# mit-han-lab/duo-attention

Hardware: NVIDIA H100
Metric: decode tok/s @512K ctx (+ prefill tok/s @128K in `prefill`), Llama-3-8B, DuoAttention 50% retrieval heads (higher is better)
Workload: dtype bf16

## Files before the change

duo_attention_b200/csrc/attn_tc.cu:

```cuda
#include <cstdlib>

#include "duo_common.cuh"

namespace duo {

constexpr int TC_THREADS = 384;
constexpr int TC_TILE = 128;
constexpr int TC_BOX_BYTES = TC_TILE * 128;
constexpr int TC_TILE_BYTES = 2 * TC_BOX_BYTES;
constexpr int TC_MAX_W = 2048;
constexpr int TC_SMEM_BYTES = 5 * TC_TILE_BYTES + TC_MAX_W + 1024;

struct TcParams {
  void* out;
  long long out_batch_stride;
  int q_len, n_q_heads, group, n_full, n_stream, batch;
  int sink, recent, W;
  long long full_len, total, lo;
  float scale_log2;
  int cache_scan;
  int n_tok_tiles;
};

__device__ __forceinline__ void wg_fence() { asm volatile("wgmma.fence.sync.aligned;" ::: "memory"); }
__device__ __forceinline__ void wg_commit() { asm volatile("wgmma.commit_group.sync.aligned;" ::: "memory"); }
template <int N>
__device__ __forceinline__ void wg_wait() {
  asm volatile("wgmma.wait_group.sync.aligned %0;" ::"n"(N) : "memory");
}
__device__ __forceinline__ void wg_fence_regs(float (&d)[64]) {
#pragma unroll
  for (int i = 0; i < 64; ++i) asm volatile("" : "+f"(d[i])::"memory");
}

__device__ __forceinline__ uint64_t make_smem_desc(uint32_t saddr, uint32_t lbo_bytes, uint32_t sbo_bytes) {
  uint64_t d = 0;
  d |= (uint64_t)((saddr >> 4) & 0x3FFF);
  d |= (uint64_t)((lbo_bytes >> 4) & 0x3FFF) << 16;
  d |= (uint64_t)((sbo_bytes >> 4) & 0x3FFF) << 32;
  d |= 1ull << 62;
  return d;
}

template <bool BF16>
__device__ __forceinline__ void wgmma_ss(float (&d)[64], uint64_t adesc, uint64_t bdesc, uint32_t accum) {
  if constexpr (BF16) {
    asm volatile(
        "{\n\t.reg .pred p;\n\tsetp.ne.b32 p, %66, 0;\n\t"
        "wgmma.mma_async.sync.aligned.m64n128k16.f32.bf16.bf16 {%0,%1,%2,%3,%4,%5,%6,%7,%8,%9,%10,%11,%12,%13,%14,%15,%16,%17,%18,%19,%20,%21,%22,%23,%24,%25,%26,%27,%28,%29,%30,%31,%32,%33,%34,%35,%36,%37,%38,%39,%40,%41,%42,%43,%44,%45,%46,%47,%48,%49,%50,%51,%52,%53,%54,%55,%56,%57,%58,%59,%60,%61,%62,%63}, %64, %65, p, 1, 1, 0, 0;\n\t}"
        : "+f"(d[0]), "+f"(d[1]), "+f"(d[2]), "+f"(d[3]), "+f"(d[4]), "+f"(d[5]), "+f"(d[6]), "+f"(d[7]), "+f"(d[8]), "+f"(d[9]), "+f"(d[10]), "+f"(d[11]), "+f"(d[12]), "+f"(d[13]), "+f"(d[14]), "+f"(d[15]), "+f"(d[16]), "+f"(d[17]), "+f"(d[18]), "+f"(d[19]), "+f"(d[20]), "+f"(d[21]), "+f"(d[22]), "+f"(d[23]), "+f"(d[24]), "+f"(d[25]), "+f"(d[26]), "+f"(d[27]), "+f"(d[28]), "+f"(d[29]), "+f"(d[30]), "+f"(d[31]), "+f"(d[32]), "+f"(d[33]), "+f"(d[34]), "+f"(d[35]), "+f"(d[36]), "+f"(d[37]), "+f"(d[38]), "+f"(d[39]), "+f"(d[40]), "+f"(d[41]), "+f"(d[42]), "+f"(d[43]), "+f"(d[44]), "+f"(d[45]), "+f"(d[46]), "+f"(d[47]), "+f"(d[48]), "+f"(d[49]), "+f"(d[50]), "+f"(d[51]), "+f"(d[52]), "+f"(d[53]), "+f"(d[54]), "+f"(d[55]), "+f"(d[56]), "+f"(d[57]), "+f"(d[58]), "+f"(d[59]), "+f"(d[60]), "+f"(d[61]), "+f"(d[62]), "+f"(d[63])
        : "l"(adesc), "l"(bdesc), "r"(accum));
  } else {
    asm volatile(
        "{\n\t.reg .pred p;\n\tsetp.ne.b32 p, %66, 0;\n\t"
        "wgmma.mma_async.sync.aligned.m64n128k16.f32.f16.f16 {%0,%1,%2,%3,%4,%5,%6,%7,%8,%9,%10,%11,%12,%13,%14,%15,%16,%17,%18,%19,%20,%21,%22,%23,%24,%25,%26,%27,%28,%29,%30,%31,%32,%33,%34,%35,%36,%37,%38,%39,%40,%41,%42,%43,%44,%45,%46,%47,%48,%49,%50,%51,%52,%53,%54,%55,%56,%57,%58,%59,%60,%61,%62,%63}, %64, %65, p, 1, 1, 0, 0;\n\t}"
        : "+f"(d[0]), "+f"(d[1]), "+f"(d[2]), "+f"(d[3]), "+f"(d[4]), "+f"(d[5]), "+f"(d[6]), "+f"(d[7]), "+f"(d[8]), "+f"(d[9]), "+f"(d[10]), "+f"(d[11]), "+f"(d[12]), "+f"(d[13]), "+f"(d[14]), "+f"(d[15]), "+f"(d[16]), "+f"(d[17]), "+f"(d[18]), "+f"(d[19]), "+f"(d[20]), "+f"(d[21]), "+f"(d[22]), "+f"(d[23]), "+f"(d[24]), "+f"(d[25]), "+f"(d[26]), "+f"(d[27]), "+f"(d[28]), "+f"(d[29]), "+f"(d[30]), "+f"(d[31]), "+f"(d[32]), "+f"(d[33]), "+f"(d[34]), "+f"(d[35]), "+f"(d[36]), "+f"(d[37]), "+f"(d[38]), "+f"(d[39]), "+f"(d[40]), "+f"(d[41]), "+f"(d[42]), "+f"(d[43]), "+f"(d[44]), "+f"(d[45]), "+f"(d[46]), "+f"(d[47]), "+f"(d[48]), "+f"(d[49]), "+f"(d[50]), "+f"(d[51]), "+f"(d[52]), "+f"(d[53]), "+f"(d[54]), "+f"(d[55]), "+f"(d[56]), "+f"(d[57]), "+f"(d[58]), "+f"(d[59]), "+f"(d[60]), "+f"(d[61]), "+f"(d[62]), "+f"(d[63])
        : "l"(adesc), "l"(bdesc), "r"(accum));
  }
}
template <bool BF16>
__device__ __forceinline__ void wgmma_rs(float (&d)[64], const uint32_t* a, uint64_t bdesc) {
  if constexpr (BF16) {
    asm volatile(
        "{\n\t.reg .pred p;\n\tsetp.ne.b32 p, %69, 0;\n\t"
        "wgmma.mma_async.sync.aligned.m64n128k16.f32.bf16.bf16 {%0,%1,%2,%3,%4,%5,%6,%7,%8,%9,%10,%11,%12,%13,%14,%15,%16,%17,%18,%19,%20,%21,%22,%23,%24,%25,%26,%27,%28,%29,%30,%31,%32,%33,%34,%35,%36,%37,%38,%39,%40,%41,%42,%43,%44,%45,%46,%47,%48,%49,%50,%51,%52,%53,%54,%55,%56,%57,%58,%59,%60,%61,%62,%63}, {%64, %65, %66, %67}, %68, p, 1, 1, 1;\n\t}"
        : "+f"(d[0]), "+f"(d[1]), "+f"(d[2]), "+f"(d[3]), "+f"(d[4]), "+f"(d[5]), "+f"(d[6]), "+f"(d[7]), "+f"(d[8]), "+f"(d[9]), "+f"(d[10]), "+f"(d[11]), "+f"(d[12]), "+f"(d[13]), "+f"(d[14]), "+f"(d[15]), "+f"(d[16]), "+f"(d[17]), "+f"(d[18]), "+f"(d[19]), "+f"(d[20]), "+f"(d[21]), "+f"(d[22]), "+f"(d[23]), "+f"(d[24]), "+f"(d[25]), "+f"(d[26]), "+f"(d[27]), "+f"(d[28]), "+f"(d[29]), "+f"(d[30]), "+f"(d[31]), "+f"(d[32]), "+f"(d[33]), "+f"(d[34]), "+f"(d[35]), "+f"(d[36]), "+f"(d[37]), "+f"(d[38]), "+f"(d[39]), "+f"(d[40]), "+f"(d[41]), "+f"(d[42]), "+f"(d[43]), "+f"(d[44]), "+f"(d[45]), "+f"(d[46]), "+f"(d[47]), "+f"(d[48]), "+f"(d[49]), "+f"(d[50]), "+f"(d[51]), "+f"(d[52]), "+f"(d[53]), "+f"(d[54]), "+f"(d[55]), "+f"(d[56]), "+f"(d[57]), "+f"(d[58]), "+f"(d[59]), "+f"(d[60]), "+f"(d[61]), "+f"(d[62]), "+f"(d[63])
        : "r"(a[0]), "r"(a[1]), "r"(a[2]), "r"(a[3]), "l"(bdesc), "r"(1));
  } else {
    asm volatile(
        "{\n\t.reg .pred p;\n\tsetp.ne.b32 p, %69, 0;\n\t"
        "wgmma.mma_async.sync.aligned.m64n128k16.f32.f16.f16 {%0,%1,%2,%3,%4,%5,%6,%7,%8,%9,%10,%11,%12,%13,%14,%15,%16,%17,%18,%19,%20,%21,%22,%23,%24,%25,%26,%27,%28,%29,%30,%31,%32,%33,%34,%35,%36,%37,%38,%39,%40,%41,%42,%43,%44,%45,%46,%47,%48,%49,%50,%51,%52,%53,%54,%55,%56,%57,%58,%59,%60,%61,%62,%63}, {%64, %65, %66, %67}, %68, p, 1, 1, 1;\n\t}"
        : "+f"(d[0]), "+f"(d[1]), "+f"(d[2]), "+f"(d[3]), "+f"(d[4]), "+f"(d[5]), "+f"(d[6]), "+f"(d[7]), "+f"(d[8]), "+f"(d[9]), "+f"(d[10]), "+f"(d[11]), "+f"(d[12]), "+f"(d[13]), "+f"(d[14]), "+f"(d[15]), "+f"(d[16]), "+f"(d[17]), "+f"(d[18]), "+f"(d[19]), "+f"(d[20]), "+f"(d[21]), "+f"(d[22]), "+f"(d[23]), "+f"(d[24]), "+f"(d[25]), "+f"(d[26]), "+f"(d[27]), "+f"(d[28]), "+f"(d[29]), "+f"(d[30]), "+f"(d[31]), "+f"(d[32]), "+f"(d[33]), "+f"(d[34]), "+f"(d[35]), "+f"(d[36]), "+f"(d[37]), "+f"(d[38]), "+f"(d[39]), "+f"(d[40]), "+f"(d[41]), "+f"(d[42]), "+f"(d[43]), "+f"(d[44]), "+f"(d[45]), "+f"(d[46]), "+f"(d[47]), "+f"(d[48]), "+f"(d[49]), "+f"(d[50]), "+f"(d[51]), "+f"(d[52]), "+f"(d[53]), "+f"(d[54]), "+f"(d[55]), "+f"(d[56]), "+f"(d[57]), "+f"(d[58]), "+f"(d[59]), "+f"(d[60]), "+f"(d[61]), "+f"(d[62]), "+f"(d[63])
        : "r"(a[0]), "r"(a[1]), "r"(a[2]), "r"(a[3]), "l"(bdesc), "r"(1));
  }
}

template <typename T>
struct TcType;
template <>
struct TcType<__nv_bfloat16> {
  static constexpr bool bf16 = true;
  __device__ static uint32_t pack(float a, float b) {
    __nv_bfloat162 v = __floats2bfloat162_rn(a, b);
    return *reinterpret_cast<uint32_t*>(&v);
  }
};
template <>
struct TcType<__half> {
  static constexpr bool bf16 = false;
  __device__ static uint32_t pack(float a, float b) {
    __half2 v = __floats2half2_rn(a, b);
    return *reinterpret_cast<uint32_t*>(&v);
  }
};

struct TcBarriers {
  uint64_t q_full;
  uint64_t k_full[2], k_empty[2], v_full[2], v_empty[2];
};

template <typename T>
__global__ void __launch_bounds__(TC_THREADS, 1)
duo_attn_tc_kernel(const __grid_constant__ CUtensorMap map_q, const __grid_constant__ CUtensorMap map_fk,
                   const __grid_constant__ CUtensorMap map_fv, const __grid_constant__ CUtensorMap map_rk,
                   const __grid_constant__ CUtensorMap map_rv, const TcParams p) {
  extern __shared__ __align__(1024) uint8_t smem_raw[];
  uint8_t* smem = reinterpret_cast<uint8_t*>((reinterpret_cast<uintptr_t>(smem_raw) + 1023) & ~uintptr_t(1023));
  __shared__ TcBarriers bars;

  uint8_t* sQ = smem;
  uint8_t* sK = smem + 1 * TC_TILE_BYTES;
  uint8_t* sV = smem + 3 * TC_TILE_BYTES;
  uint8_t* sValid = smem + 5 * TC_TILE_BYTES;

  const int tid = threadIdx.x;
  const int b = blockIdx.y;

  int x = blockIdx.x;
  const int per_kvh = p.group * p.n_tok_tiles;
  const int kvh = x / per_kvh;
  x -= kvh * per_kvh;
  const int qh = kvh * p.group + x / p.n_tok_tiles;
  const int tok0 = (p.n_tok_tiles - 1 - (x % p.n_tok_tiles)) * TC_TILE;
  const bool is_full = kvh < p.n_full;
  const int tok_hi = min(p.q_len, tok0 + TC_TILE);
  long long a0 = 0, a1, b0 = 0, b1 = 0, base;
  if (is_full) {
    base = p.full_len;
    a1 = p.full_len + tok_hi;
  } else {
    base = p.W;
    a1 = p.cache_scan;
    b0 = p.W;
    b1 = (long long)p.W + tok_hi;
  }
  const int nA = (int)((a1 - a0 + TC_TILE - 1) / TC_TILE);
  const int nB = (int)((b1 - b0 + TC_TILE - 1) / TC_TILE);
  const int n_tiles = nA + nB;
  const CUtensorMap* mk = is_full ? &map_fk : &map_rk;
  const CUtensorMap* mv = is_full ? &map_fv : &map_rv;
  const int head_coord = is_full ? (b * p.n_full + kvh) : (b * p.n_stream + (kvh - p.n_full));
  auto tile_start = [&](int i) -> long long {
    return i < nA ? a0 + (long long)i * TC_TILE : b0 + (long long)(i - nA) * TC_TILE;
  };

  if (tid == 0) {
    prefetch_tmap(&map_q);
    prefetch_tmap(mk);
    prefetch_tmap(mv);
    mbar_init(&bars.q_full, 1);
    for (int s = 0; s < 2; ++s) {
      mbar_init(&bars.k_full[s], 1);
      mbar_init(&bars.k_empty[s], 256);
      mbar_init(&bars.v_full[s], 1);
      mbar_init(&bars.v_empty[s], 256);
    }
    fence_barrier_init();
  }
  if (!is_full) {
    for (int j = tid; j < p.W; j += TC_THREADS) sValid[j] = stream_slot_valid(j, p.sink, p.recent, p.total, p.lo) ? 1 : 0;
  }
  __syncthreads();

  if (tid < 128) {
    asm volatile("setmaxnreg.dec.sync.aligned.u32 24;");
    if (tid == 0) {
      mbar_expect_tx(&bars.q_full, TC_TILE_BYTES);
      tma_load_3d(sQ, &map_q, &bars.q_full, qh * kHeadDim, tok0, b);
      tma_load_3d(sQ + TC_BOX_BYTES, &map_q, &bars.q_full, qh * kHeadDim + 64, tok0, b);
      for (int j = 0; j < n_tiles; ++j) {
        const int st = j & 1;
        const uint32_t ph = (j >> 1) & 1;
        const int j0 = (int)tile_start(j);
        mbar_wait(&bars.k_empty[st], ph ^ 1);
        mbar_expect_tx(&bars.k_full[st], TC_TILE_BYTES);
        tma_load_3d(sK + st * TC_TILE_BYTES, mk, &bars.k_full[st], 0, j0, head_coord);
        tma_load_3d(sK + st * TC_TILE_BYTES + TC_BOX_BYTES, mk, &bars.k_full[st], 64, j0, head_coord);
        mbar_wait(&bars.v_empty[st], ph ^ 1);
        mbar_expect_tx(&bars.v_full[st], TC_TILE_BYTES);
        tma_load_3d(sV + st * TC_TILE_BYTES, mv, &bars.v_full[st], 0, j0, head_coord);
        tma_load_3d(sV + st * TC_TILE_BYTES + TC_BOX_BYTES, mv, &bars.v_full[st], 64, j0, head_coord);
      }
    }
    return;
  }

  asm volatile("setmaxnreg.inc.sync.aligned.u32 240;");
  constexpr bool kBf16 = TcType<T>::bf16;
  const int wg = (tid >> 7) - 1;
  const int wt = tid & 127;
  const int quad = wt & 3;
  const int row0 = wg * 64 + (wt >> 5) * 16 + ((wt & 31) >> 2);
  const float c = p.scale_log2;
  const long long min_limit = base + tok0 + wg * 64;
  int tok[2];
  bool row_ok[2];
  long long limit[2];
#pragma unroll
  for (int i = 0; i < 2; ++i) {
    tok[i] = tok0 + row0 + 8 * i;
    row_ok[i] = tok[i] < p.q_len;
    limit[i] = base + tok[i];
  }

  const uint32_t q_addr = smem_u32(sQ) + wg * 64 * 128, k_addr = smem_u32(sK), v_addr = smem_u32(sV);
  auto issue_s = [&](float (&s)[64], int st) {
    const uint32_t ka = k_addr + st * TC_TILE_BYTES;
#pragma unroll
    for (int kk = 0; kk < 8; ++kk) {
      const uint32_t off = (kk >> 2) * TC_BOX_BYTES + (kk & 3) * 32;
      wgmma_ss<kBf16>(s, make_smem_desc(q_addr + off, 16, 1024), make_smem_desc(ka + off, 16, 1024), kk > 0);
    }
  };
  auto issue_pv = [&](float (&o)[64], const uint32_t (&pk)[32], int st) {
    const uint32_t va = v_addr + st * TC_TILE_BYTES;
#pragma unroll
    for (int kk = 0; kk < 8; ++kk) wgmma_rs<kBf16>(o, &pk[4 * kk], make_smem_desc(va + kk * 2048, TC_BOX_BYTES, 1024));
  };

  float s[64], o[64];
#pragma unroll
  for (int i = 0; i < 64; ++i) o[i] = 0.f;
  float m_run[2] = {-INFINITY, -INFINITY};
  float l_run[2] = {0.f, 0.f};

  mbar_wait(&bars.q_full, 0);
  mbar_wait(&bars.k_full[0], 0);
  wg_fence();
  issue_s(s, 0);
  wg_commit();
  wg_wait<0>();
  wg_fence_regs(s);
  mbar_arrive(&bars.k_empty[0]);

  for (int j = 0; j < n_tiles; ++j) {
    const int st = j & 1;
    const uint32_t ph = (j >> 1) & 1;
    const long long j0 = tile_start(j);
    const long long jend = (j < nA) ? a1 : b1;
    const bool cache_seg = (!is_full) && (j < nA);
    const bool need_mask = cache_seg || (j0 + TC_TILE > jend) || (j0 + TC_TILE - 1 > min_limit);
    if (need_mask) {
#pragma unroll
      for (int nb = 0; nb < 16; ++nb) {
#pragma unroll
        for (int e = 0; e < 2; ++e) {
          const long long jj = j0 + nb * 8 + quad * 2 + e;
          bool slot_ok = jj < jend;
          if (cache_seg) slot_ok = slot_ok && (jj < p.W) && (sValid[jj < p.W ? jj : 0] != 0);
#pragma unroll
          for (int i = 0; i < 2; ++i)
            if (!(slot_ok && row_ok[i] && jj <= limit[i])) s[nb * 4 + 2 * i + e] = -INFINITY;
        }
      }
    }
    uint32_t pk[32];
#pragma unroll
    for (int i = 0; i < 2; ++i) {
      float mx = -INFINITY;
#pragma unroll
      for (int nb = 0; nb < 16; ++nb) mx = fmaxf(mx, fmaxf(s[nb * 4 + 2 * i], s[nb * 4 + 2 * i + 1]));
      mx = fmaxf(mx, __shfl_xor_sync(0xffffffffu, mx, 1));
      mx = fmaxf(mx, __shfl_xor_sync(0xffffffffu, mx, 2));
      const float m_new = fmaxf(m_run[i], mx);
      const float alpha = (m_new == -INFINITY) ? 1.f : fast_exp2((m_run[i] - m_new) * c);
      const float mref_c = (m_new == -INFINITY) ? 0.f : m_new * c;
      m_run[i] = m_new;
      float rs = 0.f;
#pragma unroll
      for (int nb = 0; nb < 16; ++nb) {
        const float p0 = fast_exp2(__fmaf_rn(s[nb * 4 + 2 * i], c, -mref_c));
        const float p1 = fast_exp2(__fmaf_rn(s[nb * 4 + 2 * i + 1], c, -mref_c));
        rs += p0 + p1;
        pk[nb * 2 + i] = TcType<T>::pack(p0, p1);
        o[nb * 4 + 2 * i] *= alpha;
        o[nb * 4 + 2 * i + 1] *= alpha;
      }
      l_run[i] = l_run[i] * alpha + rs;
    }
    mbar_wait_spin(&bars.v_full[st], ph);
    wg_fence();
    issue_pv(o, pk, st);
    wg_commit();
    const bool more = j + 1 < n_tiles;
    if (more) {
      const int st1 = (j + 1) & 1;
      mbar_wait_spin(&bars.k_full[st1], ((j + 1) >> 1) & 1);
      wg_fence();
      issue_s(s, st1);
      wg_commit();
    }
    wg_wait<0>();
    wg_fence_regs(o);
    wg_fence_regs(s);
    mbar_arrive(&bars.v_empty[st]);
    if (more) mbar_arrive(&bars.k_empty[(j + 1) & 1]);
  }

  T* out_b = reinterpret_cast<T*>(p.out) + (long long)b * p.out_batch_stride;
#pragma unroll
  for (int i = 0; i < 2; ++i) {
    float l = l_run[i];
    l += __shfl_xor_sync(0xffffffffu, l, 1);
    l += __shfl_xor_sync(0xffffffffu, l, 2);
    const float inv = l > 0.f ? 1.f / l : 0.f;
    if (row_ok[i]) {
      T* dst = out_b + ((long long)tok[i] * p.n_q_heads + qh) * kHeadDim + quad * 2;
#pragma unroll
      for (int nb = 0; nb < 16; ++nb)
        *reinterpret_cast<uint32_t*>(dst + nb * 8) = TcType<T>::pack(o[nb * 4 + 2 * i] * inv, o[nb * 4 + 2 * i + 1] * inv);
    }
  }
}

typedef CUresult (*EncodeTiledFn)(CUtensorMap*, CUtensorMapDataType, cuuint32_t, void*, const cuuint64_t*,
                                  const cuuint64_t*, const cuuint32_t*, const cuuint32_t*, CUtensorMapInterleave,
                                  CUtensorMapSwizzle, CUtensorMapL2promotion, CUtensorMapFloatOOBfill);
EncodeTiledFn get_encode_fn();

bool tc_prefill_supported(const duo_layer* L, const duo_cache_state* st, int q_len) {
  (void)st;
  if (L->d.kv_format != DUO_KV_SAME) return false;
  if (q_len < TC_TILE) return false;
  if (L->d.sink + L->d.recent > TC_MAX_W) return false;
  return true;
}

int launch_attn_tc(const duo_layer* L, const duo_cache_state* st, const void* q, long long q_row_stride, void* out,
                   int q_len, float scale, cudaStream_t stream) {
  const duo_layer_desc& d = L->d;
  EncodeTiledFn fn = get_encode_fn();
  if (!fn) return DUO_ECUDA;
  CUtensorMap map_q;
  {
    cuuint64_t dims[3] = {(cuuint64_t)q_row_stride, (cuuint64_t)q_len, (cuuint64_t)d.batch};
    cuuint64_t strides[2] = {(cuuint64_t)q_row_stride * 2, (cuuint64_t)q_row_stride * 2 * (cuuint64_t)q_len};
    cuuint32_t box[3] = {64, TC_TILE, 1};
    cuuint32_t estr[3] = {1, 1, 1};
    CUresult r = fn(&map_q, d.dtype == DUO_DT_BF16 ? CU_TENSOR_MAP_DATA_TYPE_BFLOAT16 : CU_TENSOR_MAP_DATA_TYPE_FLOAT16, 3,
                    const_cast<void*>(q), dims, strides, box, estr, CU_TENSOR_MAP_INTERLEAVE_NONE,
                    CU_TENSOR_MAP_SWIZZLE_128B, CU_TENSOR_MAP_L2_PROMOTION_L2_256B, CU_TENSOR_MAP_FLOAT_OOB_FILL_NONE);
    if (r != CUDA_SUCCESS) {
      set_error("cuTensorMapEncodeTiled(q) failed with CUresult %d", (int)r);
      return DUO_ECUDA;
    }
  }
  TcParams p{};
  p.out = out;
  const int n_q = (d.n_full + d.n_stream) * d.group;
  p.out_batch_stride = (long long)q_len * n_q * kHeadDim;
  p.q_len = q_len;
  p.n_q_heads = n_q;
  p.group = d.group;
  p.n_full = d.n_full;
  p.n_stream = d.n_stream;
  p.batch = d.batch;
  p.sink = d.sink;
  p.recent = d.recent;
  p.W = d.sink + d.recent;
  p.full_len = st->full_len;
  p.total = st->total;
  p.lo = st->lo;
  p.scale_log2 = scale * 1.4426950408889634f;
  p.cache_scan = (int)std::min<long long>(p.W, st->total);
  p.n_tok_tiles = (q_len + TC_TILE - 1) / TC_TILE;
  const int grid_x = n_q * p.n_tok_tiles;
  const CUtensorMap& fk = L->has_full_maps ? L->maps.full_k128 : L->maps.ring_k128;
  const CUtensorMap& fv = L->has_full_maps ? L->maps.full_v128 : L->maps.ring_v128;
  const CUtensorMap& rk = L->has_ring_maps ? L->maps.ring_k128 : L->maps.full_k128;
  const CUtensorMap& rv = L->has_ring_maps ? L->maps.ring_v128 : L->maps.full_v128;
  if (d.dtype == DUO_DT_BF16) {
    auto kern = duo_attn_tc_kernel<__nv_bfloat16>;
    static unsigned long long attr_mask = 0;
    if (int rc = ensure_dyn_smem(kern, TC_SMEM_BYTES, &attr_mask)) return rc;
    kern<<<dim3(grid_x, d.batch), TC_THREADS, TC_SMEM_BYTES, stream>>>(map_q, fk, fv, rk, rv, p);
  } else {
    auto kern = duo_attn_tc_kernel<__half>;
    static unsigned long long attr_mask = 0;
    if (int rc = ensure_dyn_smem(kern, TC_SMEM_BYTES, &attr_mask)) return rc;
    kern<<<dim3(grid_x, d.batch), TC_THREADS, TC_SMEM_BYTES, stream>>>(map_q, fk, fv, rk, rv, p);
  }
  DUO_CUDA_TRY(cudaGetLastError());
  return DUO_OK;
}

}
```

Before: 56.49.

## Pingpong warpgroups with named barriers and overlap QK^T with PV in prefill kernel

Restructures the tensor-core prefill attention loop into a FlashAttention-3 style schedule. Each warpgroup now issues S=QK^T for tile j together with PV for tile j-1 and runs the softmax of tile j while the PV wgmma is still in flight. Named barriers alternate the two consumer warpgroups so one issues MMAs while the other does softmax. Block-to-head mapping is also changed so that consecutive blocks share the same token tile across query heads of a group, which may improve L2 reuse of K/V. The cost is more live registers (P held in s plus pk) and more complex barrier and phase bookkeeping. Decode throughput is mostly unaffected since this kernel serves prefill.

```diff
diff --git a/duo_attention_b200/csrc/attn_tc.cu b/duo_attention_b200/csrc/attn_tc.cu
--- a/duo_attention_b200/csrc/attn_tc.cu
+++ b/duo_attention_b200/csrc/attn_tc.cu
@@ -32,6 +32,8 @@
 #pragma unroll
   for (int i = 0; i < 64; ++i) asm volatile("" : "+f"(d[i])::"memory");
 }
+__device__ __forceinline__ void named_bar_sync(int id) { asm volatile("bar.sync %0, 256;" ::"r"(id) : "memory"); }
+__device__ __forceinline__ void named_bar_arrive(int id) { asm volatile("bar.arrive %0, 256;" ::"r"(id) : "memory"); }
 
 __device__ __forceinline__ uint64_t make_smem_desc(uint32_t saddr, uint32_t lbo_bytes, uint32_t sbo_bytes) {
   uint64_t d = 0;
@@ -120,8 +122,8 @@
   const int per_kvh = p.group * p.n_tok_tiles;
   const int kvh = x / per_kvh;
   x -= kvh * per_kvh;
-  const int qh = kvh * p.group + x / p.n_tok_tiles;
-  const int tok0 = (p.n_tok_tiles - 1 - (x % p.n_tok_tiles)) * TC_TILE;
+  const int qh = kvh * p.group + x % p.group;
+  const int tok0 = (p.n_tok_tiles - 1 - x / p.group) * TC_TILE;
   const bool is_full = kvh < p.n_full;
   const int tok_hi = min(p.q_len, tok0 + TC_TILE);
   long long a0 = 0, a1, b0 = 0, b1 = 0, base;
@@ -219,23 +221,14 @@
   };
 
   float s[64], o[64];
+  uint32_t pk[32];
 #pragma unroll
   for (int i = 0; i < 64; ++i) o[i] = 0.f;
   float m_run[2] = {-INFINITY, -INFINITY};
   float l_run[2] = {0.f, 0.f};
-
-  mbar_wait(&bars.q_full, 0);
-  mbar_wait(&bars.k_full[0], 0);
-  wg_fence();
-  issue_s(s, 0);
-  wg_commit();
-  wg_wait<0>();
-  wg_fence_regs(s);
-  mbar_arrive(&bars.k_empty[0]);
-
-  for (int j = 0; j < n_tiles; ++j) {
-    const int st = j & 1;
-    const uint32_t ph = (j >> 1) & 1;
+  float alpha[2];
+
+  auto softmax = [&](int j) {
     const long long j0 = tile_start(j);
     const long long jend = (j < nA) ? a1 : b1;
     const bool cache_seg = (!is_full) && (j < nA);
@@ -254,7 +247,6 @@
         }
       }
     }
-    uint32_t pk[32];
 #pragma unroll
     for (int i = 0; i < 2; ++i) {
       float mx = -INFINITY;
@@ -263,7 +255,7 @@
       mx = fmaxf(mx, __shfl_xor_sync(0xffffffffu, mx, 1));
       mx = fmaxf(mx, __shfl_xor_sync(0xffffffffu, mx, 2));
       const float m_new = fmaxf(m_run[i], mx);
-      const float alpha = (m_new == -INFINITY) ? 1.f : fast_exp2((m_run[i] - m_new) * c);
+      alpha[i] = (m_new == -INFINITY) ? 1.f : fast_exp2((m_run[i] - m_new) * c);
       const float mref_c = (m_new == -INFINITY) ? 0.f : m_new * c;
       m_run[i] = m_new;
       float rs = 0.f;
@@ -272,29 +264,74 @@
         const float p0 = fast_exp2(__fmaf_rn(s[nb * 4 + 2 * i], c, -mref_c));
         const float p1 = fast_exp2(__fmaf_rn(s[nb * 4 + 2 * i + 1], c, -mref_c));
         rs += p0 + p1;
-        pk[nb * 2 + i] = TcType<T>::pack(p0, p1);
-        o[nb * 4 + 2 * i] *= alpha;
-        o[nb * 4 + 2 * i + 1] *= alpha;
+        s[nb * 4 + 2 * i] = p0;
+        s[nb * 4 + 2 * i + 1] = p1;
       }
-      l_run[i] = l_run[i] * alpha + rs;
-    }
-    mbar_wait_spin(&bars.v_full[st], ph);
-    wg_fence();
-    issue_pv(o, pk, st);
-    wg_commit();
-    const bool more = j + 1 < n_tiles;
-    if (more) {
-      const int st1 = (j + 1) & 1;
-      mbar_wait_spin(&bars.k_full[st1], ((j + 1) >> 1) & 1);
-      wg_fence();
-      issue_s(s, st1);
-      wg_commit();
-    }
+      l_run[i] = l_run[i] * alpha[i] + rs;
+    }
+  };
+  auto rescale_pack = [&]() {
+#pragma unroll
+    for (int nb = 0; nb < 16; ++nb) {
+#pragma unroll
+      for (int i = 0; i < 2; ++i) {
+        pk[nb * 2 + i] = TcType<T>::pack(s[nb * 4 + 2 * i], s[nb * 4 + 2 * i + 1]);
+        o[nb * 4 + 2 * i] *= alpha[i];
+        o[nb * 4 + 2 * i + 1] *= alpha[i];
+      }
+    }
+  };
+  const int bar_mine = 1 + wg, bar_other = 2 - wg;
+
+  mbar_wait(&bars.q_full, 0);
+  mbar_wait(&bars.k_full[0], 0);
+  if (wg == 1) named_bar_sync(bar_mine);
+  wg_fence();
+  issue_s(s, 0);
+  wg_commit();
+  named_bar_arrive(bar_other);
+  wg_wait<0>();
+  wg_fence_regs(s);
+  mbar_arrive(&bars.k_empty[0]);
+  softmax(0);
+
+  auto retire_pv = [&](int j) {
     wg_wait<0>();
     wg_fence_regs(o);
+    if (j > 1) mbar_arrive(&bars.v_empty[j & 1]);
+    rescale_pack();
+  };
+
+  for (int j = 1; j < n_tiles; ++j) {
+    const int st = j & 1, pst = st ^ 1;
+    retire_pv(j);
+    mbar_wait_spin(&bars.k_full[st], (j >> 1) & 1);
+    mbar_wait_spin(&bars.v_full[pst], ((j - 1) >> 1) & 1);
+    named_bar_sync(bar_mine);
+    wg_fence();
+    issue_s(s, st);
+    wg_commit();
+    issue_pv(o, pk, pst);
+    wg_commit();
+    named_bar_arrive(bar_other);
+    wg_wait<1>();
     wg_fence_regs(s);
-    mbar_arrive(&bars.v_empty[st]);
-    if (more) mbar_arrive(&bars.k_empty[(j + 1) & 1]);
+    mbar_arrive(&bars.k_empty[st]);
+    softmax(j);
+  }
+
+  retire_pv(n_tiles);
+  {
+    const int pst = (n_tiles - 1) & 1;
+    mbar_wait_spin(&bars.v_full[pst], ((n_tiles - 1) >> 1) & 1);
+    named_bar_sync(bar_mine);
+    wg_fence();
+    issue_pv(o, pk, pst);
+    wg_commit();
+    if (wg == 0) named_bar_arrive(bar_other);
+    wg_wait<0>();
+    wg_fence_regs(o);
+    mbar_arrive(&bars.v_empty[pst]);
   }
 
   T* out_b = reinterpret_cast<T*>(p.out) + (long long)b * p.out_batch_stride;
```

New measurement: 56.47, median of 6. Within noise of the previous version (-0.0%).
